# placeforyiming/DistanceTransform-DepthCompletion

Hardware: AMD Instinct MI355X
Metric: DT+NN-fill frames/sec at 352x1216; achieved HBM GB/s vs peak (higher is better)
Workload: dtype u32

## Files before the change

### distancetransform-depthcompletion_amd/csrc/dtfill.hip

```cpp

#include <hip/hip_runtime.h>
#include <stdint.h>
#include <math.h>
#include <stdlib.h>
#include <type_traits>
#include "../../include/dtfill.h"

typedef uint16_t u16;
typedef uint8_t u8;
typedef unsigned long long u64;
typedef uint32_t u32;

namespace {

#include "dtfill_common.hpp"
#include "dtfill_prepass.hpp"
#include "dtfill_fused.hpp"
#include "dtfill_rows.hpp"
#include "dtfill_sky.hpp"
#include "dtfill_pts.hpp"
#include "dtfill_l2.hpp"
#include "dtfill_outlier.hpp"
#include "dtfill_gmc.hpp"
#include "dtfill_post.hpp"
// ... 69 lines not shown
}

enum { S1_MASK, S1_FRAME, S1_FUSED, S1_COLT, S1_ROWS, S1_FIN, S1_TIESX, NK_L1 };
const char *const kNamesL1[NK_L1] = {"k_mask", "k_frame", "k_fused", "k_colT", "k_rows", "k_fin", "k_tiesx"};
enum { S2_MASK, S2_FRAME, S2_WIN16, S2_WIN32, S2_FAR, S2_COLT, S2_ENV, NK_L2 };
const char *const kNamesL2[NK_L2] = {"k_mask", "k_frame", "k_l2win<10>", "k_l2win<15>", "k_l2far", "k_colT", "k_l2env"};

struct Marks {
    hipStream_t st;
    hipEvent_t *ev;
    int k = 0;
    bool ok = true;
    void at(int slot) {
        ok = ok && hipGetLastError() == hipSuccess;
        if (ev)
            for (; k <= slot; ++k) (void)hipEventRecord(ev[k], st);
    }
};

void launch_mask(const Pass &p, unsigned flags, hipStream_t st) {
    const bool vec = (p.W & 3) == 0 && (reinterpret_cast<uintptr_t>(p.x) & 15) == 0;
    const dim3 g(p.B, (p.H + 3) / 4);
    if (flags & DTFILL_FLAG_OUTLIER_REMOVAL) {
        (void)hipMemsetAsync(p.negflag, 0, (size_t)p.B * sizeof(int), st);
        auto *const filter = vec ? k_mask<1, true> : k_mask<1, false>, *const redo = vec ? k_mask<2, true> : k_mask<2, false>;
        filter<<<g, 256, 0, st>>>(p);
        redo<<<g, 256, 0, st>>>(p);
    } else {
        auto *const plain = vec ? k_mask<0, true> : k_mask<0, false>;
        plain<<<g, 256, 0, st>>>(p);
    }
}

int colT_waves(int nb) { return min(16, max(2, (nb + 3) / 4)); }

bool launch_colT(const Pass &p, const SkyArgs &sky, hipStream_t st) {
    int cw = colT_waves(p.nb);
    size_t lds = colT_lds(p.nb);
    if (sky.nblocks) {
        cw = SKY_NT / 64;
        lds = max(lds, sky_lds(sky_span_max(p.H, p.W)));
    }
    bool ok = true;
    if (lds > 48 * 1024)
        ok = hipFuncSetAttribute(reinterpret_cast<const void *>(k_colT), hipFuncAttributeMaxDynamicSharedMemorySize, (int)lds) == hipSuccess;
    const int ncol = (p.ctp + 63) / 64;
    const int fx = cw <= 4;
    k_colT<<<fx ? dim3(p.B, ncol + sky.nblocks) : dim3(ncol + sky.nblocks, p.B), 64 * cw, lds, st>>>(p, ncol, sky, fx);
    return ok;
}

int run_l1(Pass p, unsigned flags, hipStream_t st, hipEvent_t *ev) {
    const int B = p.B, H = p.H, W = p.W;
    const bool general_only = flags & DTFILL_FLAG_GENERAL_ONLY;
    const bool fused_only = flags & DTFILL_FLAG_FUSED_ONLY;
    Marks m{st, ev};
    m.at(S1_MASK);
    launch_mask(p, flags, st);
    m.at(S1_FRAME);
    auto tiling = [&](int R) {
            const int THM = F_WHM - 2 * R, TWM = F_WWM - 2 * R;
            const int nty = (H + THM - 1) / THM, ntx = (W + TWM - 1) / TWM;
            FusedTiles t;
            t.TH = (H + nty - 1) / nty;
            t.TW = (W + ntx - 1) / ntx;
            if (((t.TW + 31) & ~31) <= TWM) t.TW = (t.TW + 31) & ~31;
            t.tiles_x = ntx;
            t.nty = nty;
            t.ntiles = ntx * nty;
            return t;
        };
    const FusedTiles t16 = tiling(16), t32 = tiling(32);
    const bool epi = p.ep.row0 != 0 || p.ep.use_floor;
    const bool rowflags = !epi && !fused_only && !general_only;
    float *const out_dt_caller = p.out_dt;
    if (rowflags && !p.out_dt) p.out_dt = p.dscratch;
    k_frame<<<B, 256, 0, st>>>(p, (general_only ? 1 : 0) | (rowflags ? 4 | 8 : 0), t16.nty, t32.nty);
    m.at(S1_FUSED);
    if (!general_only) {
        auto line = [](const void *q) { return (reinterpret_cast<uintptr_t>(q) & 127) == 0; };
        const bool stream = (W & 31) == 0 && (t16.TW & 31) == 0 && (t32.TW & 31) == 0 && line(p.out_depth) && line(p.out_dt) &&
                            line(p.out_index);
        const dim3 fg(B, max(t16.ntiles, t32.ntiles));
        (stream ? k_fused<true> : k_fused<false>)<<<fg, F_NT, 0, st>>>(p.x, p.srcbits, p.wpre_s, p.rowbase_s, p.finfo, p.vlist, H, W, p.Wd, t16, t32,
                                                                      p.out_depth, p.out_dt, p.out_index, p.route, p.fflag2, p.rowfar, p.status, p.ep);
    }
    m.at(S1_COLT);
    if (!fused_only) {
        SkyArgs sky = {out_dt_caller, (W + SKY_SW - 1) / SKY_SW, 0};
        const bool sky_rides = rowflags && colT_waves(p.nb) <= SKY_NT / 64;
        if (sky_rides) sky.nblocks = sky.nstrips * ((H + SKY_RG - 1) / SKY_RG);
        m.ok = launch_colT(p, sky, st) && m.ok;
        if (rowflags && !sky_rides)
            k_sky<<<dim3(sky.nstrips * ((H + SKY_RG - 1) / SKY_RG), B), SKY_NT, sky_lds(sky_span_max(H, W)), st>>>(p, sky);
        m.at(S1_ROWS);
        const int nw8 = (W + 511) / 512, nw10 = (W + 639) / 640;
        const bool ten = nw10 * 640 < nw8 * 512;
        auto aligned = [](const void *q, uintptr_t a) { return (reinterpret_cast<uintptr_t>(q) & (a - 1)) == 0; };
        const int nwv = ten ? nw10 : nw8;
        const bool fin = p.out_depth || p.out_index;
        const float *dt = p.out_dt;
        const int ovec = (ten ? ((W & 1) == 0 && aligned(dt, 8)) : ((W & 3) == 0 && aligned(dt, 16))) |
                         (((W & 31) == 0 && dt && aligned(dt, 128)) ? 2 : 0);
        const size_t rlds = (ovec & 2) ? (size_t)W * sizeof(float) : 0;
        const int rpb = (nwv == 1 || (long long)H * B >= 16384) && nwv <= 4 ? R_RPB : 1;
        auto *const rows = rpb > 1   ? (ten ? k_rows<10, 256, true> : k_rows<8, 256, true>)
                                             : nwv <= 4 ? (ten ? k_rows<10, 256, false> : k_rows<8, 256, false>)
                                                        : (ten ? k_rows<10, 1024, false> : k_rows<8, 1024, false>);
        rows<<<dim3((H + rpb - 1) / rpb, B), 64 * nwv, rlds, st>>>(p.ct, p.ctp, p.fflag2, H, W, p.nb, p.Wp, p.planes, p.plane_bytes, p.out_dt, p.spix,
                                                                  ovec, p.rowfar, p.finfo, rpb);
        m.at(S1_FIN);
        PtsArgs pa;
        pa.ptslist = p.ptslist;
        pa.out_dt = p.out_dt;
        const int nwide = ((W + 255) / 256) * ((H + 31) / 32), ntall = ((W + 127) / 128) * ((H + 63) / 64);
        pa.tall = ntall < nwide;
        pa.tiles_x = pa.tall ? (W + 127) / 128 : (W + 255) / 256;
        pa.ntiles = rowflags ? (pa.tall ? ntall : nwide) : 0;
        const int ttx = (W + Q_TW - 1) / Q_TW;
        pa.fin_ntiles = fin ? ttx * ((H + Q_TH - 1) / Q_TH) : 0;
        if (fin || pa.ntiles) {
            const int vec = (W & 3) == 0 && aligned(p.out_depth, 16) && aligned(p.out_index, 16);
            k_fin<<<dim3(max(pa.fin_ntiles, pa.ntiles), B), Q_NT, 0, st>>>(p.planes, p.plane_bytes, p.Wp, p.fflag2, H, W, p.Wd, ttx, p.spix, p.x, p.rec,
                                                                           p.vlist, p.out_depth, p.out_index, p.status, p.finfo, p.xlist, p.xptr,
                                                                           p.planes + PL_UNRES * p.plane_bytes, vec, p.ep, p.dscratch, p.rowfar, pa);
            m.at(S1_TIESX);
            if (fin) k_tiesx<<<dim3(XL_BLOCKS, B), 256, 0, st>>>(p);
        }
    }
    m.at(NK_L1);
    return m.ok ? DTFILL_OK : DTFILL_ERR_LAUNCH;
}

int run_l2(const Pass &p, unsigned flags, hipStream_t st, hipEvent_t *ev) {
    const int B = p.B, H = p.H, W = p.W;
    Marks m{st, ev};
    m.at(S2_MASK);
    launch_mask(p, flags, st);
    m.at(S2_FRAME);
    k_frame<<<B, 256, 0, st>>>(p, ((flags & DTFILL_FLAG_GENERAL_ONLY) ? 1 : 0) | 2, 0, 0);
    m.at(S2_WIN16);
    const int ttx = (W + W2_TW - 1) / W2_TW, tty = (H + W2_TH - 1) / W2_TH;
    k_l2win<W2_R16><<<dim3(ttx * tty, B), 256, L2Win<W2_R16>::LDS, st>>>(
        p.x, p.srcbits, p.wpre_s, p.rowbase_s, p.finfo, p.vlist, p.xlist, p.route, 16, p.rowfar, p.fflag2, H, W, p.Wd, ttx, p.out_depth, p.out_dt,
        p.out_index, p.status);
    m.at(S2_WIN32);
    k_l2win<W2_R32><<<dim3(ttx * tty, B), 256, L2Win<W2_R32>::LDS, st>>>(
        p.x, p.srcbits, p.wpre_s, p.rowbase_s, p.finfo, p.vlist, p.xlist, p.route, 32, p.rowfar, p.fflag2, H, W, p.Wd, ttx, p.out_depth, p.out_dt,
        p.out_index, p.status);
    m.at(S2_FAR);
    k_l2far<<<dim3(min(256, max(16, 4096 / B)), B), 256, 0, st>>>(p);
    m.at(S2_COLT);
    m.ok = launch_colT(p, SkyArgs{}, st) && m.ok;
    m.at(S2_ENV);
    const size_t wave_lds = max(max(l2env_lds(W), (size_t)L2_PTS_MAX * 8), (size_t)(W + 2 * L2S_R) * 8);
    const int ntile = ((H + PT_T - 1) / PT_T) * ((W + PT_T - 1) / PT_T);
    if (4 * wave_lds <= 64 * 1024) {
        const int nrowblk = (H + 3) / 4;
        k_l2env<4><<<dim3(B, nrowblk + (ntile + 3) / 4), 256, 4 * wave_lds, st>>>(p.x, p.ct, p.ctp, p.nb, p.rec, p.Wd, p.finfo, p.vlist, p.route,
                                                                                  p.rowfar, p.srclist(), H, W, nrowblk, wave_lds, 1, p.out_depth,
                                                                                  p.out_dt, p.out_index, p.status);
    } else {
        if (wave_lds > 48 * 1024)
            m.ok = m.ok && hipFuncSetAttribute(reinterpret_cast<const void *>(k_l2env<1>), hipFuncAttributeMaxDynamicSharedMemorySize,
                                               (int)l2env_lds(8192)) == hipSuccess;
        k_l2env<1><<<dim3(B, H + (ntile + 7) / 8), 64, wave_lds, st>>>(p.x, p.ct, p.ctp, p.nb, p.rec, p.Wd, p.finfo, p.vlist, p.route, p.rowfar,
                                                                       p.srclist(), H, W, H, wave_lds, 8, p.out_depth, p.out_dt, p.out_index,
// ... 120 lines not shown
    if (metric == DTFILL_METRIC_L2 && k >= 0 && k < NK_L2) return kNamesL2[k];
    return "";
}

int dtfill_batch_timed(const float *x, int B, int H, int W, float src_thr, float val_thr, int metric,
                       float *out_depth, float *out_dt, int32_t *out_index, int32_t *frame_status,
                       void *workspace, size_t ws_bytes, void *stream, unsigned flags, float *kernel_ms) {
    int rc = check_args(x, B, H, W, metric, out_depth, out_dt, out_index, workspace, ws_bytes, flags);
    if (rc != DTFILL_OK) return rc;
    if (!kernel_ms) return DTFILL_ERR_NULL;
    const int nk = dtfill_num_kernels(metric);
    static_assert(NK_L2 <= NK_L1, "event array");
    hipEvent_t ev[NK_L1 + 1];
    for (int k = 0; k <= nk; ++k)
        if (hipEventCreate(&ev[k]) != hipSuccess) {
            while (k-- > 0) (void)hipEventDestroy(ev[k]);
            return DTFILL_ERR_NO_DEVICE;
        }
    rc = run(make_pass(x, B, H, W, src_thr, val_thr, out_depth, out_dt, out_index, frame_status, workspace), metric, flags, stream, ev);
    (void)hipEventSynchronize(ev[nk]);
    for (int k = 0; k < nk; ++k) (void)hipEventElapsedTime(&kernel_ms[k], ev[k], ev[k + 1]);
    for (int k = 0; k <= nk; ++k) (void)hipEventDestroy(ev[k]);
    return rc;
}

int dtfill_pass_stats(const void *workspace, size_t ws_bytes, int B, int H, int W, int metric, long long *out_px, void *stream) {
    if (!workspace || !out_px) return DTFILL_ERR_NULL;
    if (!shape_ok(B, H, W)) return DTFILL_ERR_SHAPE;
    if (metric != DTFILL_METRIC_L1_CV && metric != DTFILL_METRIC_L2) return DTFILL_ERR_METRIC;
    if (ws_bytes < dtfill_workspace_bytes(B, H, W, metric) || ((uintptr_t)workspace & 255)) return DTFILL_ERR_WORKSPACE;
    hipStream_t st = static_cast<hipStream_t>(stream);
    if (hipMemsetAsync(out_px, 0, DTFILL_STATS_N * sizeof(long long), st) != hipSuccess) return DTFILL_ERR_LAUNCH;
    k_stats<<<B, 256, 0, st>>>(carve(const_cast<void *>(workspace), B, H, W), metric == DTFILL_METRIC_L2 ? 1 : 0, out_px);
    return hipGetLastError() == hipSuccess ? DTFILL_OK : DTFILL_ERR_LAUNCH;
}

int dtfill_crop_floor(const float *x, int B, int H, int W, int r0, int r1, int c0, int c1, int use_floor, float floor_,
                      float *out, void *stream) {
    if (!x || !out) return DTFILL_ERR_NULL;
    if (B < 1 || H < 1 || W < 1 || (long long)B * H * W >= (1ll << 31) || B > 65535 || H > 65535) return DTFILL_ERR_SHAPE;
    if (r0 < 0 || r1 > H || r0 >= r1 || c0 < 0 || c1 > W || c0 >= c1) return DTFILL_ERR_SHAPE;
    const int OH = r1 - r0, OW = c1 - c0;
    k_crop_floor<<<dim3(min((OW + 255) / 256, 8), OH, B), 256, 0, static_cast<hipStream_t>(stream)>>>(
        x, H, W, r0, c0, OH, OW, use_floor, floor_, out);
    return hipGetLastError() == hipSuccess ? DTFILL_OK : DTFILL_ERR_LAUNCH;
}

int dtfill_png16(const float *x, int B, int H, int W, int pad_top, int use_floor, float floor_, float lo, float hi,
                 float scale, uint16_t *out, void *stream) {
    if (!x || !out) return DTFILL_ERR_NULL;
    if (B < 1 || H < 1 || W < 1 || pad_top < 0 || (long long)B * ((long long)H + pad_top) * W >= (1ll << 31) || B > 65535 ||
        H + pad_top > 65535)
        return DTFILL_ERR_SHAPE;
    k_png16<<<dim3(min((W + 255) / 256, 8), H + pad_top, B), 256, 0, static_cast<hipStream_t>(stream)>>>(
        x, H, W, pad_top, use_floor, floor_, lo, hi, scale, out);
    return hipGetLastError() == hipSuccess ? DTFILL_OK : DTFILL_ERR_LAUNCH;
}

size_t dtfill_metrics_workspace_bytes(int B) {
    if (B < 1 || B > 65535) return 0;
    return (size_t)B * M_NB * M_NS * sizeof(double);
}

int dtfill_metrics(const float *output, const float *target, int B, long long n, int kind, double *out, void *workspace,
                   size_t ws_bytes, void *stream) {
    if (!output || !target || !out || !workspace) return DTFILL_ERR_NULL;
    if (B < 1 || B > 65535 || n < 1 || n >= (1ll << 40)) return DTFILL_ERR_SHAPE;
    if (kind != DTFILL_METRICS_KITTI && kind != DTFILL_METRICS_NYU) return DTFILL_ERR_METRIC;
    if (ws_bytes < dtfill_metrics_workspace_bytes(B)) return DTFILL_ERR_WORKSPACE;
    hipStream_t st = static_cast<hipStream_t>(stream);
    double *part = static_cast<double *>(workspace);
    if (kind == DTFILL_METRICS_KITTI) {
        k_metrics_part<0><<<dim3(M_NB, B), 256, 0, st>>>(output, target, n, part);
        k_metrics_final<0><<<B, 64, 0, st>>>(part, M_NB, out);
    } else {
        k_metrics_part<1><<<dim3(M_NB, B), 256, 0, st>>>(output, target, n, part);
        k_metrics_final<1><<<B, 64, 0, st>>>(part, M_NB, out);
    }
    return hipGetLastError() == hipSuccess ? DTFILL_OK : DTFILL_ERR_LAUNCH;
}

}

#ifdef PTS_PROF
extern "C" int dtfill_pts_prof(unsigned long long *out8, int reset) {
    unsigned long long z[12] = {0, 0, 0, 0, 0, 0, 0, 0, 0, 0, 0, 0};
    if (hipMemcpyFromSymbol(out8, HIP_SYMBOL(g_pts_prof), sizeof(z)) != hipSuccess) return -1;
    if (reset && hipMemcpyToSymbol(HIP_SYMBOL(g_pts_prof), z, sizeof(z)) != hipSuccess) return -1;
    return 0;
}
#endif
```

### distancetransform-depthcompletion_amd/csrc/dtfill_fused.hpp

```cpp
#pragma once

constexpr int F_WHM = 128;
constexpr int F_WWM = 192;
constexpr int F_NT = 256;
constexpr int F_P = 196;
constexpr int F_NWD = 6;
constexpr int F_HW = 3;
constexpr int F_RS = 7;
constexpr int F_RROWS = F_WHM + 4;
constexpr int F_RPLANE = F_RROWS * F_RS;
constexpr int F_RING = 1 + 4 * 2 * F_RPLANE;
constexpr int F_EB = 8;
constexpr int F_NONE = 2 * 63;
static_assert(F_WWM == 32 * F_NWD, "window width must be six words");
static_assert(F_RING * 4 >= F_WHM * F_P + 256 * 8, "s_par and the un-slicing table must fit in the ring's memory");
static_assert((F_WHM * F_P) % 8 == 0 && F_WHM * F_P >= 4 * (1 + 4 * F_RPLANE), "the table is 8-byte aligned and lies behind the planes of P1b");

#define ENC_F(t) (((TAP_DI(t) + 2) << 3) | (TAP_DJ(t) + 2))

template <int DJ>
__device__ __forceinline__ u32 hshift(const u32 (&a)[5], int i) {
    if (DJ == 0) return a[i + 1];
    if (DJ > 0) return __builtin_amdgcn_alignbit(a[i + 2], a[i + 1], DJ);
    return __builtin_amdgcn_alignbit(a[i + 1], a[i], 32 + DJ);
}

template <int DJ, int ENC>
__device__ __forceinline__ void tap_step(const u32 (&src)[5], u32 (&taken)[F_HW], u32 (&C)[6][F_HW]) {
#pragma unroll
    for (int i = 0; i < F_HW; ++i) {
        const u32 cand = hshift<DJ>(src, i);
        const u32 sel = cand & ~taken[i];
        taken[i] |= cand;
#pragma unroll
        for (int j = 0; j < 6; ++j)
            if (ENC & (1 << j)) C[j][i] |= sel;
    }
}

template <int DJ, int WGT, int ENC>
__device__ __forceinline__ void bwd_tap(const u32 (&a0)[5], const u32 (&a1)[5], const u32 (&a2)[5], const u32 (&dv)[5],
                                        const u32 (&b0)[F_HW], const u32 (&b1)[F_HW], const u32 (&b2)[F_HW],
                                        u32 (&taken)[F_HW], u32 (&C)[6][F_HW]) {
#pragma unroll
    for (int i = 0; i < F_HW; ++i) {
        const u32 x0 = hshift<DJ>(a0, i), x1 = hshift<DJ>(a1, i), x2 = hshift<DJ>(a2, i);
        u32 s0, s1, s2;
        if (WGT == 1) {
            s0 = ~x0; s1 = x1 ^ x0; s2 = x2 ^ (x1 & x0);
        } else if (WGT == 2) {
            s0 = x0; s1 = ~x1; s2 = x2 ^ x1;
        } else {
            s0 = ~x0; s1 = ~(x1 ^ x0); s2 = x2 ^ (x1 | x0);
        }
        const u32 m = ~((s0 ^ b0[i]) | (s1 ^ b1[i]) | (s2 ^ b2[i])) & hshift<DJ>(dv, i);
        const u32 sel = m & ~taken[i];
        taken[i] |= m;
#pragma unroll
        for (int j = 0; j < 6; ++j)
            if (ENC & (1 << j)) C[j][i] |= sel;
    }
}

__device__ __forceinline__ u32 mul_u24_opaque(u32 a, u32 b) {
    u32 r;
    asm("v_mul_u32_u24 %0, %1, %2" : "=v"(r) : "v"(a), "v"(b));
    return r;
}

__device__ __forceinline__ void ring_load5(const u32 *__restrict__ ring, int slot, int plane, int row, int wb,
                                           u32 (&a)[5]) {
    const u32 *p = ring + 1 + (slot * 2 + plane) * F_RPLANE + row * F_RS + wb - 1;
#pragma unroll
    for (int i = 0; i < 5; ++i) a[i] = p[i];
}
__device__ __forceinline__ void ring_store3(u32 *__restrict__ ring, int slot, int plane, int row, int wb,
                                            const u32 (&w)[F_HW]) {
    u32 *p = ring + 1 + (slot * 2 + plane) * F_RPLANE + row * F_RS + wb;
#pragma unroll
    for (int i = 0; i < F_HW; ++i) p[i] = w[i];
}

template <int FR, int NT, bool EPI, bool STREAM>
__device__ __forceinline__ bool fused_walk_epilogue(
    const u8 *__restrict__ s_par, const short *__restrict__ s_tab, const uint2 *__restrict__ s_rw, int b, int H,
    int W, int th, int tw, int r0, int c0, int wr0, int wc0, int sh, const float *__restrict__ x,
    const float *__restrict__ vlist,
    int *__restrict__ finfo, float *__restrict__ out_depth, float *__restrict__ out_dt,
    int32_t *__restrict__ out_index, int *__restrict__ frame_status, const DepthEpilogue ep, u32 *__restrict__ rowflag) {
    const size_t fo = (size_t)b * H * W;
    const int nval = finfo[b * FI_STRIDE + FI_NVAL];
    const int misaligned = finfo[b * FI_STRIDE + FI_MISALIGNED];
    const float *gbase = misaligned ? vlist + fo : x + fo;
    float *od = out_depth ? out_depth + (size_t)b * (H - ep.row0) * W : nullptr, *ot = out_dt ? out_dt + fo : nullptr;
    const u32 dcrop = (u32)(ep.row0 * W) << 2;
    constexpr bool plain = !EPI;
    int32_t *oi = out_index ? out_index + fo : nullptr;
    const char *tab = reinterpret_cast<const char *>(s_tab);
    const int src_base = wr0 * W + wc0;
    const u32 last_px = (u32)(H * W - 1);
    bool overflow = false;
    const int nslots = ((th + F_EB - 1) / F_EB) * tw;
    const float inv_tw = 1.0f / (float)tw;
    const u32 w4 = (u32)W << 2;
    int p_lab[F_EB], p_dd[F_EB];
    u32 p_opix[F_EB];
    float p_val[F_EB];
    u32 p_ok = 0;
    auto retire = [&]() {
#pragma unroll
        for (int e = 0; e < F_EB; ++e) {
            if (!((p_ok >> e) & 1u)) continue;
            auto put = [](auto *p, auto v) {
                if constexpr (STREAM)
                    __builtin_nontemporal_store(v, p);
                else
                    *p = v;
            };
            if (oi) put(reinterpret_cast<int32_t *>(reinterpret_cast<char *>(oi) + p_opix[e]), p_lab[e]);
            if (ot) put(reinterpret_cast<float *>(reinterpret_cast<char *>(ot) + p_opix[e]), (float)p_dd[e]);
            if (od && plain) {
                put(reinterpret_cast<float *>(reinterpret_cast<char *>(od) + p_opix[e]), p_val[e]);
            } else if (od && p_opix[e] >= dcrop) {
                *reinterpret_cast<float *>(reinterpret_cast<char *>(od) + (p_opix[e] - dcrop)) = depth_epilogue(p_val[e], ep);
            }
        }
    };
    for (int sb = 0; sb < nslots; sb += NT) {
        int pos[F_EB], code[F_EB];
        u32 home[F_EB];
        u32 opix[F_EB];
        u32 ok = 0;
        {
            const int L = sb + (int)threadIdx.x, Lc = min(L, nslots - 1);
            const int g = (int)(((float)Lc + 0.5f) * inv_tw);
            const int tc = Lc - __mul24(g, tw), trb = g * F_EB;
            const u32 home0 = (u32)(FR + trb) << 16 | (u32)(FR + tc);
            const u32 opix0 = (u32)(__mul24(r0 + trb, W) + c0 + tc) << 2;
            const int pos0 = __mul24(FR + trb, F_P) + FR + tc;
            const int nv = L < nslots ? th - trb : 0;
#pragma unroll
            for (int e = 0; e < F_EB; ++e) {
                const bool valid = e < nv;
                home[e] = home0 + ((u32)e << 16);
                opix[e] = opix0 + (u32)e * w4;
                pos[e] = pos0 + e * F_P;
                code[e] = s_par[pos[e]];
                ok |= (valid && code[e] != F_NONE) ? (1u << e) : 0u;
                overflow |= valid && code[e] == F_NONE;
            }
        }
        for (int hop = 0; hop < FR + 2; hop += 2) {
            int step[F_EB];
#pragma unroll
            for (int e = 0; e < F_EB; ++e) step[e] = *reinterpret_cast<const short *>(tab + code[e]);
            int moving = 0;
#pragma unroll
            for (int e = 0; e < F_EB; ++e) moving |= step[e];
            if (!__any(moving != 0)) break;
#pragma unroll
            for (int e = 0; e < F_EB; ++e) pos[e] += step[e];
#pragma unroll
            for (int e = 0; e < F_EB; ++e) code[e] = s_par[pos[e]];
#pragma unroll
            for (int e = 0; e < F_EB; ++e) step[e] = *reinterpret_cast<const short *>(tab + code[e]);
#pragma unroll
            for (int e = 0; e < F_EB; ++e) pos[e] += step[e];
#pragma unroll
            for (int e = 0; e < F_EB; ++e) code[e] = s_par[pos[e]];
        }
        int lab[F_EB], dd[F_EB];
        u32 goff[F_EB];
        bool bad = false;
#pragma unroll
        for (int e = 0; e < F_EB; ++e) {
            static_assert(F_P == 196 && F_WHM * F_P < (1 << 15), "the reciprocal below is F_P's");
            const int pr_ = (int)(__umul24((u32)pos[e], 5350u) >> 20), pc_ = pos[e] - __mul24(pr_, F_P);
            dd[e] = (int)__builtin_amdgcn_sad_u16((u32)pr_ << 16 | (u32)pc_, home[e], 0u);
            const int bitpos = sh + pc_;
            const uint2 rw = s_rw[pr_ * 8 + (bitpos >> 5)];
            lab[e] = (int)rw.y + __popc(rw.x & ((1u << (bitpos & 31)) - 1u)) + 1;
            if (!misaligned) {
                goff[e] = min((u32)(src_base + __mul24(pr_, W) + pc_), last_px) << 2;
            } else {
                const int idx = lab[e] - 1;
                const bool oob = idx >= nval;
                bad |= ((ok >> e) & 1u) && oob;
                goff[e] = (oob ? 0u : min((u32)idx, last_px)) << 2;
            }
        }
        if (bad && out_depth) atomicOr(frame_status + b, DTFILL_FRAME_INDEX_ERROR);
        retire();
#pragma unroll
        for (int e = 0; e < F_EB; ++e) {
            p_val[e] = *reinterpret_cast<const float *>(reinterpret_cast<const char *>(gbase) + goff[e]);
            p_lab[e] = lab[e];
            p_dd[e] = dd[e];
            p_opix[e] = opix[e];
        }
        p_ok = ok;
    }
    retire();
    const bool any = __any(overflow);
    if (any && !EPI) {
        for (int L = threadIdx.x; L < nslots; L += NT) {
            const int g = L / tw, tc = L - g * tw;
            for (int tr = g * F_EB; tr < min(g * F_EB + F_EB, th); ++tr)
                if (s_par[__mul24(FR + tr, F_P) + FR + tc] == F_NONE) {
                    rowflag[(size_t)b * H + r0 + tr] = 1u;
                    const int s0 = finfo[b * FI_STRIDE + FI_SKY0];
                    if (s0 > 0 && (r0 + tr == s0 || r0 + tr == s0 + 1)) finfo[b * FI_STRIDE + FI_SKY] = 0;
                }
        }
    }
    return any;
}

struct FusedTiles {
    int TH, TW, tiles_x, ntiles, nty;
};

template <int FR, bool EPI, bool STREAM>
__device__ __forceinline__ void fused_body(bool premarked,
    const float *__restrict__ x, const u64 *__restrict__ srcbits, const u16 *__restrict__ wpre_s,
    const u32 *__restrict__ rowbase_s, int *__restrict__ finfo, const float *__restrict__ vlist,
    int H, int W, int Wd, int nty, int TW, int tiles_x, float *__restrict__ out_depth,
    float *__restrict__ out_dt, int32_t *__restrict__ out_index,
    int *__restrict__ fflag, u32 *__restrict__ rowfar, int *__restrict__ frame_status, const DepthEpilogue ep, u32 *__restrict__ s_ring, uint2 *__restrict__ s_rw,
    short *__restrict__ s_tab, u32 (*__restrict__ s_any)[F_NT / 64]) {
    const int tid = threadIdx.x;
    const int b = blockIdx.x;
    const int ty = blockIdx.y / tiles_x, tx = blockIdx.y - ty * tiles_x;
    const int tbase = finfo[b * FI_STRIDE + FI_TR0];
    const int TH = (H - tbase + nty - 1) / nty;
    int r0 = tbase + ty * TH;
    const int c0 = tx * TW;
    int th = min(TH, H - r0);
    const int tw = min(TW, W - c0);
    if (th <= 0) return;
    if (premarked) {
        const u32 *rowflag = rowfar + (size_t)b * H;
        if (tid == 0) {
            s_any[0][0] = 0xFFFFFFFFu;
            s_any[0][1] = 0u;
        }
        __syncthreads();
        if (tid < th && rowflag[r0 + tid] == 0u) {
            atomicMin(&s_any[0][0], (u32)tid);
            atomicMax(&s_any[0][1], (u32)tid + 1u);
        }
        __syncthreads();
        const u32 lo = s_any[0][0], hi = s_any[0][1];
        if (hi == 0u) return;
        r0 += (int)lo;
        th = (int)(hi - lo);
    }
    const int wr0 = r0 - FR, wc0 = c0 - FR;
    const int WH = th + 2 * FR, WW = tw + 2 * FR;
    const int ca = max(0, -wc0), cb = min(WW, W - wc0);
    const int w0 = wc0 >> 6;
    const int sh = wc0 - 64 * w0;

    const int r = tid & (F_WHM - 1);
    const int hf = tid >> 7;
    const int wb = F_HW * hf;
    u32 M[F_HW], D[F_HW], TM[F_HW];
    {
        const int gi = wr0 + r;
        const bool rowin = r < WH && gi >= 0 && gi < H;
        const int bit0 = sh + 96 * hf;
        const int kw = bit0 >> 6;
        u32 g[7];
#pragma unroll
        for (int k = 0; k < 3; ++k) {
            const int kk = kw + k;
            const int w = w0 + kk;
            u64 sb = 0;
            u32 rk = 0;
            if (rowin && kk < 4 && w >= 0 && w < Wd) {
                const size_t wi = ((size_t)b * H + gi) * Wd + w;
                sb = srcbits[wi];
                rk = rowbase_s[(size_t)b * H + gi] + wpre_s[wi];
            }
            g[2 * k] = (u32)sb;
            g[2 * k + 1] = (u32)(sb >> 32);
            const bool mine = hf == 0 ? kk < 2 : (kk >= 2 && kk < 4);
            if (mine) {
                s_rw[r * 8 + 2 * kk] = make_uint2((u32)sb, rk);
                s_rw[r * 8 + 2 * kk + 1] = make_uint2((u32)(sb >> 32), rk + (u32)__popc((u32)sb));
            }
        }
        g[6] = 0;
        const int s6 = bit0 & 63;
        const bool hi = s6 & 32;
        const int s5 = s6 & 31;
#pragma unroll
        for (int i = 0; i < F_HW; ++i) {
            const u32 lo_w = hi ? g[i + 1] : g[i], hi_w = hi ? g[i + 2] : g[i + 1];
            const u32 word = s5 ? __builtin_amdgcn_alignbit(hi_w, lo_w, s5) : lo_w;
            const int lo = max(ca - 32 * (wb + i), 0), up = min(cb - 32 * (wb + i), 32);
            u32 m = 0;
            if (rowin && up > lo) m = (up >= 32 ? 0xFFFFFFFFu : ((1u << up) - 1u)) & ~((1u << lo) - 1u);
            M[i] = m;
            D[i] = word & m;
            const int tlo = max(FR - 32 * (wb + i), 0), tup = min(FR + tw - 32 * (wb + i), 32);
            u32 tm = 0;
            if (r >= FR && r < FR + th && tup > tlo) tm = (tup >= 32 ? 0xFFFFFFFFu : ((1u << tup) - 1u)) & ~((1u << tlo) - 1u);
            TM[i] = tm;
        }
    }
    for (int k = tid; k < F_RING; k += F_NT) s_ring[k] = 0;
    if (tid < 64) {
        const int hi = tid >> 3, lo = tid & 7;
        s_tab[tid] = (hi <= 4 && lo <= 4) ? (short)((hi - 2) * F_P + (lo - 2)) : (short)0;
    }
    __syncthreads();
    ring_store3(s_ring, 0, 0, r + 2, wb, D);
    ring_store3(s_ring, 0, 1, r + 2, wb, D);
    u32 C[6][F_HW];
#pragma unroll
    for (int j = 0; j < 6; ++j)
#pragma unroll
        for (int i = 0; i < F_HW; ++i) C[j][i] = ((18 >> j) & 1) ? D[i] : 0u;
    u32 Dup[F_HW], Ddn[F_HW];
    u32 Dl = 0, Dr = 0;
#pragma unroll
    for (int i = 0; i < F_HW; ++i) Dup[i] = Ddn[i] = 0;
    __syncthreads();

    u32 P0[F_HW], P1[F_HW], P2[F_HW];
#pragma unroll
    for (int i = 0; i < F_HW; ++i) P0[i] = P1[i] = P2[i] = 0;
    for (int t = 1; t <= FR; ++t) {
        const int s1 = (t - 1) & 3, s2 = (t - 2) & 3, s3 = (t - 3) & 3, sw = t & 3;
        u32 nb[5], e1[5], l1[5], taken[F_HW], Et[F_HW], Lt[F_HW];
        ring_load5(s_ring, s1, 0, r + 2, wb, e1);
        Dl |= e1[0];
        Dr |= e1[4];
        ring_load5(s_ring, s1, 0, r + 1, wb, nb);
#pragma unroll
        for (int i = 0; i < F_HW; ++i) Dup[i] |= nb[i + 1];
        u32 e1d[5];
        ring_load5(s_ring, s1, 0, r + 3, wb, e1d);
        bool nonempty = false;
        {
            const u32 dd[5] = {Dl, D[0], D[1], D[2], Dr};
#pragma unroll
            for (int i = 0; i < F_HW; ++i) {
                Ddn[i] |= e1d[i + 1];
                const u32 dil = hshift<1>(dd, i) | hshift<-1>(dd, i) | Dup[i] | Ddn[i];
                Et[i] = dil & ~D[i] & M[i];
                taken[i] = ~Et[i];
                nonempty |= Et[i] != 0;
            }
        }
        ring_load5(s_ring, s3, 1, r + 0, wb, nb);
        tap_step<-1, ENC_F(0)>(nb, taken, C);
        tap_step<1, ENC_F(1)>(nb, taken, C);
        {
            u32 l3[5], l2[5];
            ring_load5(s_ring, s3, 1, r + 1, wb, l3);
            ring_load5(s_ring, s2, 1, r + 1, wb, l2);
            ring_load5(s_ring, s1, 1, r + 1, wb, nb);
            tap_step<-2, ENC_F(2)>(l3, taken, C);
            tap_step<-1, ENC_F(3)>(l2, taken, C);
            tap_step<0, ENC_F(4)>(nb, taken, C);
            tap_step<1, ENC_F(5)>(l2, taken, C);
            tap_step<2, ENC_F(6)>(l3, taken, C);
        }
        ring_load5(s_ring, s1, 1, r + 2, wb, l1);
        tap_step<-1, ENC_F(7)>(l1, taken, C);
        {
            const u32 m0 = (t & 1) ? 0xFFFFFFFFu : 0u, m1 = (t & 2) ? 0xFFFFFFFFu : 0u, m2 = (t & 4) ? 0xFFFFFFFFu : 0u;
#pragma unroll
            for (int i = 0; i < F_HW; ++i) {
                Lt[i] = taken[i] & Et[i];
                P0[i] |= Et[i] & m0;
                P1[i] |= Et[i] & m1;
                P2[i] |= Et[i] & m2;
            }
        }
#pragma unroll
        for (int i = 0; i < F_HW; ++i) D[i] |= Et[i];
        ring_store3(s_ring, sw, 0, r + 2, wb, Et);
        ring_store3(s_ring, sw, 1, r + 2, wb, Lt);
        {
            bool open = false;
#pragma unroll
            for (int i = 0; i < F_HW; ++i) open |= (TM[i] & ~D[i]) != 0;
            const u32 flags = (__any(nonempty) ? 1u : 0u) | (__any(open) ? 2u : 0u);
            if ((tid & 63) == 0) s_any[t & 1][tid >> 6] = flags;
            __syncthreads();
            u32 any = 0;
#pragma unroll
            for (int w = 0; w < F_NT / 64; ++w) any |= s_any[t & 1][w];
            if (any != 3u) break;
        }
    }
    __syncthreads();
    uint2 *s_lut = reinterpret_cast<uint2 *>(reinterpret_cast<u8 *>(s_ring) + F_WHM * F_P);
    s_lut[tid] = make_uint2((((u32)tid & 15u) * 0x00204081u) & 0x01010101u, (((u32)tid >> 4) * 0x00204081u) & 0x01010101u);
    ring_store3(s_ring, 0, 0, r + 2, wb, P0);
    ring_store3(s_ring, 0, 1, r + 2, wb, P1);
    ring_store3(s_ring, 1, 0, r + 2, wb, P2);
    ring_store3(s_ring, 1, 1, r + 2, wb, D);
    __syncthreads();
    {
        u32 taken[F_HW], a0[5], a1[5], a2[5], dv[5];
#pragma unroll
        for (int i = 0; i < F_HW; ++i) {
            const u32 live = C[0][i] | C[1][i] | C[2][i] | C[3][i] | C[4][i] | C[5][i];
            taken[i] = ~(D[i] & ~live);
        }
        auto row4 = [&](int row) {
            ring_load5(s_ring, 0, 0, row, wb, a0);
            ring_load5(s_ring, 0, 1, row, wb, a1);
            ring_load5(s_ring, 1, 0, row, wb, a2);
            ring_load5(s_ring, 1, 1, row, wb, dv);
        };
        row4(r + 4);
        bwd_tap<1, 3, 36 - ENC_F(0)>(a0, a1, a2, dv, P0, P1, P2, taken, C);
        bwd_tap<-1, 3, 36 - ENC_F(1)>(a0, a1, a2, dv, P0, P1, P2, taken, C);
        row4(r + 3);
        bwd_tap<2, 3, 36 - ENC_F(2)>(a0, a1, a2, dv, P0, P1, P2, taken, C);
        bwd_tap<1, 2, 36 - ENC_F(3)>(a0, a1, a2, dv, P0, P1, P2, taken, C);
        bwd_tap<0, 1, 36 - ENC_F(4)>(a0, a1, a2, dv, P0, P1, P2, taken, C);
        bwd_tap<-1, 2, 36 - ENC_F(5)>(a0, a1, a2, dv, P0, P1, P2, taken, C);
        bwd_tap<-2, 3, 36 - ENC_F(6)>(a0, a1, a2, dv, P0, P1, P2, taken, C);
        row4(r + 2);
        bwd_tap<1, 1, 36 - ENC_F(7)>(a0, a1, a2, dv, P0, P1, P2, taken, C);
    }

    u8 *s_par = reinterpret_cast<u8 *>(s_ring);
    __syncthreads();
    {
        u32 *prow = reinterpret_cast<u32 *>(s_par + r * F_P) + wb * 8;
#pragma unroll
        for (int i = 0; i < F_HW; ++i) {
            u32 cj[6];
#pragma unroll
            for (int j = 0; j < 6; ++j) cj[j] = C[j][i] | ~D[i];
#pragma unroll
            for (int q = 0; q < 4; ++q) {
                u32 lo = 0, hi = 0;
#pragma unroll
                for (int j = 0; j < 6; ++j) {
                    const uint2 sp = s_lut[(cj[j] >> (8 * q)) & 0xFFu];
                    lo |= sp.x << (j + 1);
                    hi |= sp.y << (j + 1);
                }
                prow[i * 8 + 2 * q] = lo;
                prow[i * 8 + 2 * q + 1] = hi;
            }
        }
    }
    __syncthreads();

    const bool overflow = fused_walk_epilogue<FR, F_NT, EPI, STREAM>(s_par, s_tab, s_rw, b, H, W, th, tw, r0, c0, wr0, wc0, sh, x, vlist,
                                                        finfo, out_depth, out_dt, out_index, frame_status, ep, rowfar);
    if (overflow && (threadIdx.x & 63) == 0) {
        fflag[b] = EPI ? 2 : 1;
        atomicOr(frame_status + b, DTFILL_FRAME_GENERAL_PATH);
    }
}

constexpr size_t F_OFF_RW = (sizeof(u32) * F_RING + 15) & ~(size_t)15, F_OFF_TAB = F_OFF_RW + sizeof(uint2) * F_WHM * 8, F_OFF_ANY = F_OFF_TAB + sizeof(short) * 64,
                 F_LDS_OWN = F_OFF_ANY + sizeof(u32) * 2 * (F_NT / 64);
constexpr size_t F_LDS = F_LDS_OWN;

template <bool STREAM>
__global__ __launch_bounds__(F_NT, 4) void k_fused(
    const float *__restrict__ x, const u64 *__restrict__ srcbits, const u16 *__restrict__ wpre_s,
    const u32 *__restrict__ rowbase_s, int *__restrict__ finfo, const float *__restrict__ vlist,
    int H, int W, int Wd, FusedTiles t16, FusedTiles t32, float *__restrict__ out_depth,
    float *__restrict__ out_dt, int32_t *__restrict__ out_index,
    const int *__restrict__ route, int *__restrict__ fflag, u32 *__restrict__ rowfar, int *__restrict__ frame_status, const DepthEpilogue ep) {
    __shared__ __attribute__((aligned(16))) unsigned char s_raw[F_LDS];
    u32 *s_ring = reinterpret_cast<u32 *>(s_raw);
    uint2 *s_rw = reinterpret_cast<uint2 *>(s_raw + F_OFF_RW);
    short *s_tab = reinterpret_cast<short *>(s_raw + F_OFF_TAB);
    u32(*s_any)[F_NT / 64] = reinterpret_cast<u32(*)[F_NT / 64]>(s_raw + F_OFF_ANY);
    const int rt = route[blockIdx.x];
    if (rt == ROUTE_POINTS) return;
    const int r = rt > 0 ? (rt & 0xFF) : 0;
    const bool pre = rt > 0 && (rt & ROUTE_PREMARK);
    const bool epi = ep.row0 != 0 || ep.use_floor;
#define FUSED_CALL(FR_, EPI_, T_)                                                                                        \
    fused_body<FR_, EPI_, STREAM && !(EPI_)>(pre, x, srcbits, wpre_s, rowbase_s, finfo, vlist, H, W, Wd, T_.nty, T_.TW, T_.tiles_x, out_depth, out_dt, \
                          out_index, fflag, rowfar, frame_status, ep, s_ring, s_rw, s_tab, s_any)
    if (r == 16 && (int)blockIdx.y < t16.ntiles) {
        if (epi)
            FUSED_CALL(16, true, t16);
        else
            FUSED_CALL(16, false, t16);
    } else if (r == 32 && (int)blockIdx.y < t32.ntiles) {
        if (epi)
            FUSED_CALL(32, true, t32);
        else
            FUSED_CALL(32, false, t32);
    }
#undef FUSED_CALL
}
```

Baseline: 368,700.

## Slim fused walk epilogue registers and hoist EPI into kernel template

The walk epilogue now writes the index and distance outputs right after the walk instead of holding per-element label, distance and pixel-offset arrays until the next retire. Only the depth values stay deferred, and they use a single base offset. A wave-uniform 'all slots valid' flag lets stores skip per-element predication. The +1 label bias moves into the s_rw table, and EPI becomes a kernel template parameter so each instantiation compiles only one epilogue variant. An optional FUSED_PROF cycle profiler is also added. The aim is lower register pressure, less code, and fewer branches, at the cost of a different store ordering.

```diff
diff --git a/distancetransform-depthcompletion_amd/csrc/dtfill.hip b/distancetransform-depthcompletion_amd/csrc/dtfill.hip
--- a/distancetransform-depthcompletion_amd/csrc/dtfill.hip
+++ b/distancetransform-depthcompletion_amd/csrc/dtfill.hip
@@ -175,7 +175,7 @@
         const bool stream = (W & 31) == 0 && (t16.TW & 31) == 0 && (t32.TW & 31) == 0 && line(p.out_depth) && line(p.out_dt) &&
                             line(p.out_index);
         const dim3 fg(B, max(t16.ntiles, t32.ntiles));
-        (stream ? k_fused<true> : k_fused<false>)<<<fg, F_NT, 0, st>>>(p.x, p.srcbits, p.wpre_s, p.rowbase_s, p.finfo, p.vlist, H, W, p.Wd, t16, t32,
+        (epi ? k_fused<false, true> : stream ? k_fused<true, false> : k_fused<false, false>)<<<fg, F_NT, 0, st>>>(p.x, p.srcbits, p.wpre_s, p.rowbase_s, p.finfo, p.vlist, H, W, p.Wd, t16, t32,
                                                                       p.out_depth, p.out_dt, p.out_index, p.route, p.fflag2, p.rowfar, p.status, p.ep);
     }
     m.at(S1_COLT);
@@ -462,6 +462,23 @@
 
 }
 
+#ifdef FUSED_PROF
+extern "C" int dtfill_fused_prof(unsigned long long *out16, int reset) {
+    static unsigned long long h[F_PROF_SLOTS][16];
+    if (hipMemcpyFromSymbol(h, HIP_SYMBOL(g_fused_prof), sizeof(h)) != hipSuccess) return -1;
+    for (int k = 0; k < 16; ++k) {
+        out16[k] = 0;
+        for (int i = 0; i < F_PROF_SLOTS; ++i) out16[k] += h[i][k];
+    }
+    if (reset) {
+        for (auto &r : h)
+            for (auto &v : r) v = 0;
+        if (hipMemcpyToSymbol(HIP_SYMBOL(g_fused_prof), h, sizeof(h)) != hipSuccess) return -1;
+    }
+    return 0;
+}
+#endif
+
 #ifdef PTS_PROF
 extern "C" int dtfill_pts_prof(unsigned long long *out8, int reset) {
     unsigned long long z[12] = {0, 0, 0, 0, 0, 0, 0, 0, 0, 0, 0, 0};
diff --git a/distancetransform-depthcompletion_amd/csrc/dtfill_fused.hpp b/distancetransform-depthcompletion_amd/csrc/dtfill_fused.hpp
--- a/distancetransform-depthcompletion_amd/csrc/dtfill_fused.hpp
+++ b/distancetransform-depthcompletion_amd/csrc/dtfill_fused.hpp
@@ -68,6 +68,30 @@
     return r;
 }
 
+#ifdef FUSED_PROF
+constexpr int F_PROF_SLOTS = 8192;
+__device__ unsigned long long g_fused_prof[F_PROF_SLOTS][16];
+struct FusedProf {
+    unsigned long long t[8] = {}, n[8] = {}, tprev = __builtin_readcyclecounter();
+    __device__ void mark(int k) {
+        const unsigned long long t_ = __builtin_readcyclecounter();
+        t[k] += t_ - tprev;
+        tprev = t_;
+    }
+    __device__ void flush() {
+        const int slot = ((blockIdx.y * gridDim.x + blockIdx.x) * (blockDim.x >> 6) + (threadIdx.x >> 6)) % F_PROF_SLOTS;
+        if ((threadIdx.x & 63) == 0)
+            for (int k = 0; k < 8; ++k) {
+                atomicAdd(&g_fused_prof[slot][k], t[k]);
+                atomicAdd(&g_fused_prof[slot][8 + k], n[k]);
+            }
+    }
+};
+#define FPROF(...) __VA_ARGS__
+#else
+#define FPROF(...)
+#endif
+
 __device__ __forceinline__ void ring_load5(const u32 *__restrict__ ring, int slot, int plane, int row, int wb,
                                            u32 (&a)[5]) {
     const u32 *p = ring + 1 + (slot * 2 + plane) * F_RPLANE + row * F_RS + wb - 1;
@@ -87,63 +111,65 @@
     int W, int th, int tw, int r0, int c0, int wr0, int wc0, int sh, const float *__restrict__ x,
     const float *__restrict__ vlist,
     int *__restrict__ finfo, float *__restrict__ out_depth, float *__restrict__ out_dt,
-    int32_t *__restrict__ out_index, int *__restrict__ frame_status, const DepthEpilogue ep, u32 *__restrict__ rowflag) {
+    int32_t *__restrict__ out_index, int *__restrict__ frame_status, const DepthEpilogue ep, u32 *__restrict__ rowflag
+    FPROF(, FusedProf &prof)) {
     const size_t fo = (size_t)b * H * W;
     const int nval = finfo[b * FI_STRIDE + FI_NVAL];
     const int misaligned = finfo[b * FI_STRIDE + FI_MISALIGNED];
     const float *gbase = misaligned ? vlist + fo : x + fo;
     float *od = out_depth ? out_depth + (size_t)b * (H - ep.row0) * W : nullptr, *ot = out_dt ? out_dt + fo : nullptr;
     const u32 dcrop = (u32)(ep.row0 * W) << 2;
-    constexpr bool plain = !EPI;
     int32_t *oi = out_index ? out_index + fo : nullptr;
     const char *tab = reinterpret_cast<const char *>(s_tab);
+    auto step_of = [&](int c) { return (int)*reinterpret_cast<const short *>(tab + c); };
     const int src_base = wr0 * W + wc0;
     const u32 last_px = (u32)(H * W - 1);
     bool overflow = false;
+    auto put = [](auto *p, auto v) {
+        if constexpr (STREAM)
+            __builtin_nontemporal_store(v, p);
+        else
+            *p = v;
+    };
     const int nslots = ((th + F_EB - 1) / F_EB) * tw;
     const float inv_tw = 1.0f / (float)tw;
     const u32 w4 = (u32)W << 2;
-    int p_lab[F_EB], p_dd[F_EB];
-    u32 p_opix[F_EB];
     float p_val[F_EB];
-    u32 p_ok = 0;
+    u32 p_opix = 0, p_ok = 0;
+    bool p_full = false;
     auto retire = [&]() {
-#pragma unroll
-        for (int e = 0; e < F_EB; ++e) {
-            if (!((p_ok >> e) & 1u)) continue;
-            auto put = [](auto *p, auto v) {
-                if constexpr (STREAM)
-                    __builtin_nontemporal_store(v, p);
-                else
-                    *p = v;
-            };
-            if (oi) put(reinterpret_cast<int32_t *>(reinterpret_cast<char *>(oi) + p_opix[e]), p_lab[e]);
-            if (ot) put(reinterpret_cast<float *>(reinterpret_cast<char *>(ot) + p_opix[e]), (float)p_dd[e]);
-            if (od && plain) {
-                put(reinterpret_cast<float *>(reinterpret_cast<char *>(od) + p_opix[e]), p_val[e]);
-            } else if (od && p_opix[e] >= dcrop) {
-                *reinterpret_cast<float *>(reinterpret_cast<char *>(od) + (p_opix[e] - dcrop)) = depth_epilogue(p_val[e], ep);
-            }
+        if (!od) return;
+        auto st = [&](int e) {
+            const u32 o = p_opix + (u32)e * w4;
+            if constexpr (!EPI)
+                put(reinterpret_cast<float *>(reinterpret_cast<char *>(od) + o), p_val[e]);
+            else if (o >= dcrop)
+                *reinterpret_cast<float *>(reinterpret_cast<char *>(od) + (o - dcrop)) = depth_epilogue(p_val[e], ep);
+        };
+        if (p_full) {
+#pragma unroll
+            for (int e = 0; e < F_EB; ++e) st(e);
+        } else {
+#pragma unroll
+            for (int e = 0; e < F_EB; ++e)
+                if ((p_ok >> e) & 1u) st(e);
         }
     };
     for (int sb = 0; sb < nslots; sb += NT) {
-        int pos[F_EB], code[F_EB];
-        u32 home[F_EB];
-        u32 opix[F_EB];
-        u32 ok = 0;
+        int pos[F_EB], step[F_EB], code[F_EB];
+        u32 ok = 0, home0, opix0;
+        FPROF(prof.mark(5); ++prof.n[2]);
         {
             const int L = sb + (int)threadIdx.x, Lc = min(L, nslots - 1);
             const int g = (int)(((float)Lc + 0.5f) * inv_tw);
             const int tc = Lc - __mul24(g, tw), trb = g * F_EB;
-            const u32 home0 = (u32)(FR + trb) << 16 | (u32)(FR + tc);
-            const u32 opix0 = (u32)(__mul24(r0 + trb, W) + c0 + tc) << 2;
+            home0 = (u32)(FR + trb) << 16 | (u32)(FR + tc);
+            opix0 = (u32)(__mul24(r0 + trb, W) + c0 + tc) << 2;
             const int pos0 = __mul24(FR + trb, F_P) + FR + tc;
             const int nv = L < nslots ? th - trb : 0;
 #pragma unroll
             for (int e = 0; e < F_EB; ++e) {
                 const bool valid = e < nv;
-                home[e] = home0 + ((u32)e << 16);
-                opix[e] = opix0 + (u32)e * w4;
                 pos[e] = pos0 + e * F_P;
                 code[e] = s_par[pos[e]];
                 ok |= (valid && code[e] != F_NONE) ? (1u << e) : 0u;
@@ -151,55 +177,75 @@
             }
         }
         for (int hop = 0; hop < FR + 2; hop += 2) {
-            int step[F_EB];
-#pragma unroll
-            for (int e = 0; e < F_EB; ++e) step[e] = *reinterpret_cast<const short *>(tab + code[e]);
+#pragma unroll
+            for (int e = 0; e < F_EB; ++e) step[e] = step_of(code[e]);
             int moving = 0;
 #pragma unroll
             for (int e = 0; e < F_EB; ++e) moving |= step[e];
             if (!__any(moving != 0)) break;
+            FPROF(++prof.n[5]);
 #pragma unroll
             for (int e = 0; e < F_EB; ++e) pos[e] += step[e];
 #pragma unroll
             for (int e = 0; e < F_EB; ++e) code[e] = s_par[pos[e]];
 #pragma unroll
-            for (int e = 0; e < F_EB; ++e) step[e] = *reinterpret_cast<const short *>(tab + code[e]);
+            for (int e = 0; e < F_EB; ++e) step[e] = step_of(code[e]);
 #pragma unroll
             for (int e = 0; e < F_EB; ++e) pos[e] += step[e];
 #pragma unroll
             for (int e = 0; e < F_EB; ++e) code[e] = s_par[pos[e]];
         }
-        int lab[F_EB], dd[F_EB];
+        FPROF(prof.mark(4); for (int e = 0; e < F_EB; ++e) prof.n[3] += __popcll(__ballot((ok >> e) & 1u)));
+        int pr[F_EB], pc[F_EB];
         u32 goff[F_EB];
-        bool bad = false;
+        int lab[F_EB];
 #pragma unroll
         for (int e = 0; e < F_EB; ++e) {
             static_assert(F_P == 196 && F_WHM * F_P < (1 << 15), "the reciprocal below is F_P's");
-            const int pr_ = (int)(__umul24((u32)pos[e], 5350u) >> 20), pc_ = pos[e] - __mul24(pr_, F_P);
-            dd[e] = (int)__builtin_amdgcn_sad_u16((u32)pr_ << 16 | (u32)pc_, home[e], 0u);
-            const int bitpos = sh + pc_;
-            const uint2 rw = s_rw[pr_ * 8 + (bitpos >> 5)];
-            lab[e] = (int)rw.y + __popc(rw.x & ((1u << (bitpos & 31)) - 1u)) + 1;
-            if (!misaligned) {
-                goff[e] = min((u32)(src_base + __mul24(pr_, W) + pc_), last_px) << 2;
-            } else {
+            pr[e] = (int)(__umul24((u32)pos[e], 5350u) >> 20);
+            pc[e] = pos[e] - __mul24(pr[e], F_P);
+            const int bitpos = sh + pc[e];
+            const uint2 rw = s_rw[pr[e] * 8 + (bitpos >> 5)];
+            lab[e] = (int)rw.y + __popc(rw.x & ((1u << (bitpos & 31)) - 1u));
+        }
+        if (!misaligned) {
+#pragma unroll
+            for (int e = 0; e < F_EB; ++e) goff[e] = min((u32)(src_base + __mul24(pr[e], W) + pc[e]), last_px) << 2;
+        } else {
+            bool bad = false;
+#pragma unroll
+            for (int e = 0; e < F_EB; ++e) {
                 const int idx = lab[e] - 1;
                 const bool oob = idx >= nval;
                 bad |= ((ok >> e) & 1u) && oob;
                 goff[e] = (oob ? 0u : min((u32)idx, last_px)) << 2;
             }
-        }
-        if (bad && out_depth) atomicOr(frame_status + b, DTFILL_FRAME_INDEX_ERROR);
+            if (bad && out_depth) atomicOr(frame_status + b, DTFILL_FRAME_INDEX_ERROR);
+        }
         retire();
 #pragma unroll
-        for (int e = 0; e < F_EB; ++e) {
-            p_val[e] = *reinterpret_cast<const float *>(reinterpret_cast<const char *>(gbase) + goff[e]);
-            p_lab[e] = lab[e];
-            p_dd[e] = dd[e];
-            p_opix[e] = opix[e];
-        }
+        for (int e = 0; e < F_EB; ++e) p_val[e] = *reinterpret_cast<const float *>(reinterpret_cast<const char *>(gbase) + goff[e]);
+        p_opix = opix0;
         p_ok = ok;
-    }
+        p_full = __all(ok == (1u << F_EB) - 1u);
+        if (oi || ot) {
+            auto st = [&](int e) {
+                const u32 o = opix0 + (u32)e * w4;
+                if (oi) put(reinterpret_cast<int32_t *>(reinterpret_cast<char *>(oi) + o), lab[e]);
+                if (ot) put(reinterpret_cast<float *>(reinterpret_cast<char *>(ot) + o),
+                            (float)__builtin_amdgcn_sad_u16((u32)pr[e] << 16 | (u32)pc[e], home0 + ((u32)e << 16), 0u));
+            };
+            if (p_full) {
+#pragma unroll
+                for (int e = 0; e < F_EB; ++e) st(e);
+            } else {
+#pragma unroll
+                for (int e = 0; e < F_EB; ++e)
+                    if ((ok >> e) & 1u) st(e);
+            }
+        }
+    }
+    FPROF(prof.mark(5));
     retire();
     const bool any = __any(overflow);
     if (any && !EPI) {
@@ -255,6 +301,7 @@
         r0 += (int)lo;
         th = (int)(hi - lo);
     }
+    FPROF(FusedProf prof; prof.n[0] = 1);
     const int wr0 = r0 - FR, wc0 = c0 - FR;
     const int WH = th + 2 * FR, WW = tw + 2 * FR;
     const int ca = max(0, -wc0), cb = min(WW, W - wc0);
@@ -286,8 +333,8 @@
             g[2 * k + 1] = (u32)(sb >> 32);
             const bool mine = hf == 0 ? kk < 2 : (kk >= 2 && kk < 4);
             if (mine) {
-                s_rw[r * 8 + 2 * kk] = make_uint2((u32)sb, rk);
-                s_rw[r * 8 + 2 * kk + 1] = make_uint2((u32)(sb >> 32), rk + (u32)__popc((u32)sb));
+                s_rw[r * 8 + 2 * kk] = make_uint2((u32)sb, rk + 1u);
+                s_rw[r * 8 + 2 * kk + 1] = make_uint2((u32)(sb >> 32), rk + 1u + (u32)__popc((u32)sb));
             }
         }
         g[6] = 0;
@@ -327,11 +374,13 @@
 #pragma unroll
     for (int i = 0; i < F_HW; ++i) Dup[i] = Ddn[i] = 0;
     __syncthreads();
+    FPROF(prof.mark(0));
 
     u32 P0[F_HW], P1[F_HW], P2[F_HW];
 #pragma unroll
     for (int i = 0; i < F_HW; ++i) P0[i] = P1[i] = P2[i] = 0;
     for (int t = 1; t <= FR; ++t) {
+        FPROF(++prof.n[1]);
         const int s1 = (t - 1) & 3, s2 = (t - 2) & 3, s3 = (t - 3) & 3, sw = t & 3;
         u32 nb[5], e1[5], l1[5], taken[F_HW], Et[F_HW], Lt[F_HW];
         ring_load5(s_ring, s1, 0, r + 2, wb, e1);
@@ -397,6 +446,7 @@
             if (any != 3u) break;
         }
     }
+    FPROF(prof.mark(1));
     __syncthreads();
     uint2 *s_lut = reinterpret_cast<uint2 *>(reinterpret_cast<u8 *>(s_ring) + F_WHM * F_P);
     s_lut[tid] = make_uint2((((u32)tid & 15u) * 0x00204081u) & 0x01010101u, (((u32)tid >> 4) * 0x00204081u) & 0x01010101u);
@@ -431,6 +481,7 @@
         bwd_tap<1, 1, 36 - ENC_F(7)>(a0, a1, a2, dv, P0, P1, P2, taken, C);
     }
 
+    FPROF(prof.mark(2));
     u8 *s_par = reinterpret_cast<u8 *>(s_ring);
     __syncthreads();
     {
@@ -455,20 +506,22 @@
         }
     }
     __syncthreads();
+    FPROF(prof.mark(3));
 
     const bool overflow = fused_walk_epilogue<FR, F_NT, EPI, STREAM>(s_par, s_tab, s_rw, b, H, W, th, tw, r0, c0, wr0, wc0, sh, x, vlist,
-                                                        finfo, out_depth, out_dt, out_index, frame_status, ep, rowfar);
+                                                        finfo, out_depth, out_dt, out_index, frame_status, ep, rowfar FPROF(, prof));
     if (overflow && (threadIdx.x & 63) == 0) {
         fflag[b] = EPI ? 2 : 1;
         atomicOr(frame_status + b, DTFILL_FRAME_GENERAL_PATH);
     }
+    FPROF(prof.mark(6); prof.flush());
 }
 
 constexpr size_t F_OFF_RW = (sizeof(u32) * F_RING + 15) & ~(size_t)15, F_OFF_TAB = F_OFF_RW + sizeof(uint2) * F_WHM * 8, F_OFF_ANY = F_OFF_TAB + sizeof(short) * 64,
                  F_LDS_OWN = F_OFF_ANY + sizeof(u32) * 2 * (F_NT / 64);
 constexpr size_t F_LDS = F_LDS_OWN;
 
-template <bool STREAM>
+template <bool STREAM, bool EPI>
 __global__ __launch_bounds__(F_NT, 4) void k_fused(
     const float *__restrict__ x, const u64 *__restrict__ srcbits, const u16 *__restrict__ wpre_s,
     const u32 *__restrict__ rowbase_s, int *__restrict__ finfo, const float *__restrict__ vlist,
@@ -484,20 +537,12 @@
     if (rt == ROUTE_POINTS) return;
     const int r = rt > 0 ? (rt & 0xFF) : 0;
     const bool pre = rt > 0 && (rt & ROUTE_PREMARK);
-    const bool epi = ep.row0 != 0 || ep.use_floor;
-#define FUSED_CALL(FR_, EPI_, T_)                                                                                        \
-    fused_body<FR_, EPI_, STREAM && !(EPI_)>(pre, x, srcbits, wpre_s, rowbase_s, finfo, vlist, H, W, Wd, T_.nty, T_.TW, T_.tiles_x, out_depth, out_dt, \
+#define FUSED_CALL(FR_, T_)                                                                                        \
+    fused_body<FR_, EPI, STREAM>(pre, x, srcbits, wpre_s, rowbase_s, finfo, vlist, H, W, Wd, T_.nty, T_.TW, T_.tiles_x, out_depth, out_dt, \
                           out_index, fflag, rowfar, frame_status, ep, s_ring, s_rw, s_tab, s_any)
-    if (r == 16 && (int)blockIdx.y < t16.ntiles) {
-        if (epi)
-            FUSED_CALL(16, true, t16);
-        else
-            FUSED_CALL(16, false, t16);
-    } else if (r == 32 && (int)blockIdx.y < t32.ntiles) {
-        if (epi)
-            FUSED_CALL(32, true, t32);
-        else
-            FUSED_CALL(32, false, t32);
-    }
+    if (r == 16 && (int)blockIdx.y < t16.ntiles)
+        FUSED_CALL(16, t16);
+    else if (r == 32 && (int)blockIdx.y < t32.ntiles)
+        FUSED_CALL(32, t32);
 #undef FUSED_CALL
 }
```

Result: faster. 384,700, median of 6 (+4.3%).
